# bezirganyan/m2-mixer

Measured on AMD Instinct MI355X. Metric: training samples/sec AV-MNIST M2-Mixer-B bf16, higher is better.
Workload: dtype bf16

## Files before the change

### include/m2mixer.h

```cpp
#ifndef M2MIXER_H
#define M2MIXER_H

#include <stdint.h>

#ifdef __cplusplus
extern "C" {
#endif

#define M2M_ABI_VERSION 18
#define M2M_MAX_BLOCKS 8
#define M2M_ROWS_PER_WG 16

#define M2M_SPLIT_GPART 1472

#define M2M_PREC_BF16 0
#define M2M_PREC_F32 1

typedef struct m2m_block {
    const float* ln1_w;
    const float* ln1_b;
    const float* tok_w1;
    const float* tok_b1;
    const float* tok_w2;
    const float* tok_b2;
// ... 101 lines not shown
int m2m_towers_forward_embeds(const m2m_tower* const* towers, const m2m_tower_io* io, int ntowers,
                              const m2m_embed* const* embeds, const float* const* inputs, const m2m_step_head* head,
                              int B, int training, uint32_t seed, uint32_t step, const uint32_t* step_dev, void* stream);

int m2m_tower_backward(const m2m_tower* t, int B, const float* d_out, int64_t d_out_sample_stride,
                       const float* d_pooled, float* d_x0, int64_t d_x0_sample_stride,
                       uint32_t seed, uint32_t step, const uint32_t* step_dev, void* stream);
typedef struct m2m_tower_gio {
    const float* d_out; int64_t d_out_sample_stride;
    const float* d_pooled;
    float* d_x0; int64_t d_x0_sample_stride;
} m2m_tower_gio;
int m2m_towers_backward(const m2m_tower* const* towers, const m2m_tower_gio* io, int ntowers, int B,
                        uint32_t seed, uint32_t step, const uint32_t* step_dev, void* stream);
int m2m_tower_wgrad(const m2m_tower* t, int B, uint32_t seed, uint32_t step, const uint32_t* step_dev, void* stream);
int m2m_wgrad_form(const m2m_tower* t, int B);
int m2m_split_form(const m2m_tower* a, const m2m_tower* b, int B, int training);
int m2m_towers_wgrad(const m2m_tower* const* towers, const m2m_tower* const* dev_towers, int ntowers,
                     const m2m_embed* const* embeds, const float* const* inputs, const float* const* d_x0s,
                     const m2m_tower* const* embed_towers, int nembeds,
                     int B, uint32_t seed, uint32_t step, const uint32_t* step_dev, void* stream);
int m2m_wgrad_groups(const m2m_tower* t, int B);
int m2m_embeds_wgrad_form(const m2m_embed* const* embeds, const m2m_tower* const* embed_towers, int nembeds, int B);
int m2m_wgrad_slot_groups(const m2m_tower* const* towers, int ntowers, int B);
int m2m_wgrad_fold(const m2m_tower* t, void* stream);
int m2m_embed_wgrad(const m2m_embed* e, const float* input, const float* d_x0, int B, void* stream);
int m2m_embeds_wgrad(const m2m_embed* const* embeds, const float* const* inputs, const float* const* d_x0s, int nembeds, int B,
                     void* stream);

typedef struct m2m_head {
    const float* pooled;
    const float* w;
    const float* b;
    float* g_w;
    float* g_b;
    float* d_pooled;
    float weight;
    float* g_part;
    const float* tokens;
    int64_t tok_sample_stride;
    int32_t ntok;
} m2m_head;
int m2m_heads_part_tiles(int B);
int m2m_heads_ce(const m2m_head* heads, int nheads, const int64_t* labels, int B, int D, int K,
                 float* logits, float* losses, int32_t* preds, int zero_losses, void* stream);

// ... 120 lines not shown
```

### m2_mixer_amd/_lib.py

```python
from __future__ import annotations

import ctypes as C
import os
import subprocess

_HERE = os.path.dirname(os.path.abspath(__file__))
LIB_PATH = os.environ.get("M2M_LIB_PATH", os.path.join(_HERE, "libm2mixer.so"))
CSRC = os.path.join(_HERE, "csrc")

ABI_VERSION = 18
MAX_BLOCKS = 8
ROWS_PER_WG = 16
HCHN_PAD = 4096
SPLIT_ROWS = 128
SPLIT_MAX = 8
SPLIT_GPART = 1472
PREC_BF16, PREC_F32 = 0, 1
PREC_BY_NAME = {"bf16": PREC_BF16, "fp32": PREC_F32, "f32": PREC_F32}

_fp = C.c_void_p


class Block(C.Structure):
    PARAMS = ["ln1_w", "ln1_b", "tok_w1", "tok_b1", "tok_w2", "tok_b2", "ln2_w", "ln2_b",
# ... 89 lines not shown
    "m2m_tower_backward_heads": (C.c_int, [C.POINTER(Tower), C.c_int, C.POINTER(Head), C.c_int, C.c_int, _fp, C.c_int, _fp, _fp, _fp, _fp,
                                           C.c_int64, C.c_uint32, C.c_uint32, _fp, _fp]),
    "m2m_tower_wgrad": (C.c_int, [C.POINTER(Tower), C.c_int, C.c_uint32, C.c_uint32, _fp, _fp]),
    "m2m_towers_can_group": (C.c_int, [C.POINTER(Tower), C.POINTER(Tower), C.c_int]),
    "m2m_towers_forward": (C.c_int, [C.POINTER(C.POINTER(Tower)), C.POINTER(TowerIO), C.c_int, C.c_int, C.c_int, C.c_uint32,
                                     C.c_uint32, _fp, _fp]),
    "m2m_towers_forward_embeds_ok": (C.c_int, [C.POINTER(C.POINTER(Tower)), C.c_int, C.POINTER(C.POINTER(Embed)), C.c_int]),
    "m2m_towers_forward_embeds": (C.c_int, [C.POINTER(C.POINTER(Tower)), C.POINTER(TowerIO), C.c_int, C.POINTER(C.POINTER(Embed)),
                                            C.POINTER(_fp), C.POINTER(StepHead), C.c_int, C.c_int, C.c_uint32, C.c_uint32, _fp, _fp]),
    "m2m_towers_backward": (C.c_int, [C.POINTER(C.POINTER(Tower)), C.POINTER(TowerGIO), C.c_int, C.c_int, C.c_uint32, C.c_uint32,
                                      _fp, _fp]),
    "m2m_towers_wgrad": (C.c_int, [C.POINTER(C.POINTER(Tower)), C.POINTER(_fp), C.c_int, C.POINTER(C.POINTER(Embed)), C.POINTER(_fp),
                                   C.POINTER(_fp), C.POINTER(C.POINTER(Tower)), C.c_int, C.c_int, C.c_uint32, C.c_uint32, _fp, _fp]),
    "m2m_towers_wgrad_heads": (C.c_int, [C.POINTER(C.POINTER(Tower)), C.POINTER(_fp), C.c_int, C.POINTER(C.POINTER(Embed)), C.POINTER(_fp),
                                         C.POINTER(_fp), C.POINTER(C.POINTER(Tower)), C.c_int, C.c_int, C.c_uint32, C.c_uint32, _fp,
                                         C.POINTER(Head), C.c_int, C.c_int, _fp]),
    "m2m_towers_wgrad_tail": (C.c_int, [C.POINTER(C.POINTER(Tower)), C.POINTER(_fp), C.c_int, C.POINTER(C.POINTER(Embed)), C.POINTER(_fp),
                                        C.POINTER(_fp), C.POINTER(C.POINTER(Tower)), C.c_int, C.c_int, C.c_uint32, C.c_uint32, _fp,
                                        C.POINTER(Head), C.c_int, C.c_int, _fp, _fp]),
    "m2m_heads_part_tiles": (C.c_int, [C.c_int]),
    "m2m_wgrad_form": (C.c_int, [C.POINTER(Tower), C.c_int]),
    "m2m_split_form": (C.c_int, [C.POINTER(Tower), C.POINTER(Tower), C.c_int, C.c_int]),
    "m2m_embeds_wgrad_form": (C.c_int, [C.POINTER(C.POINTER(Embed)), C.POINTER(C.POINTER(Tower)), C.c_int, C.c_int]),
    "m2m_wgrad_groups": (C.c_int, [C.POINTER(Tower), C.c_int]),
    "m2m_wgrad_slot_groups": (C.c_int, [C.POINTER(C.POINTER(Tower)), C.c_int, C.c_int]),
    "m2m_wgrad_fold": (C.c_int, [C.POINTER(Tower), _fp]),
    "m2m_adam_step_ranges": (C.c_int, [_fp, _fp, _fp, _fp, _fp, C.c_int64, _fp, C.c_float, C.c_float, C.c_float, C.c_float,
                                       C.c_float, C.c_int, C.POINTER(GradRange), C.c_int, _fp]),
    "m2m_counter_add": (C.c_int, [_fp, C.c_uint32, _fp]),
    "m2m_embed_wgrad": (C.c_int, [C.POINTER(Embed), _fp, _fp, C.c_int, _fp]),
    "m2m_embeds_wgrad": (C.c_int, [C.POINTER(C.POINTER(Embed)), C.POINTER(_fp), C.POINTER(_fp), C.c_int, C.c_int, _fp]),
    "m2m_embeds_forward": (C.c_int, [C.POINTER(C.POINTER(Embed)), C.POINTER(_fp), C.POINTER(_fp), C.POINTER(C.c_int), C.POINTER(C.c_int64),
                                     C.c_int, C.c_int, C.POINTER(StepHead), _fp]),
    "m2m_embed_fwd_splits": (C.c_int, [C.POINTER(Embed)]),
    "m2m_heads_ce": (C.c_int, [C.POINTER(Head), C.c_int, _fp, C.c_int, C.c_int, C.c_int, _fp, _fp, _fp, C.c_int, _fp]),
    "m2m_step_prologue": (C.c_int, [_fp, _fp, _fp, C.c_int, _fp]),
    "m2m_heads_bce": (C.c_int, [C.POINTER(Head), C.c_int, _fp, _fp, C.c_int, C.c_int, C.c_int, _fp, _fp, _fp, C.c_int, _fp]),
    "m2m_heads_ce_w": (C.c_int, [C.POINTER(Head), C.c_int, _fp, C.c_int, C.c_int, C.c_int, _fp, _fp, _fp, C.c_int, _fp, _fp]),
    "m2m_heads_bce_w": (C.c_int, [C.POINTER(Head), C.c_int, _fp, _fp, C.c_int, C.c_int, C.c_int, _fp, _fp, _fp, C.c_int, _fp, _fp]),
    "m2m_fusion_forward": (C.c_int, [C.c_int, _fp, _fp, _fp, C.c_int64, _fp]),
    "m2m_fusion_backward": (C.c_int, [C.c_int, _fp, _fp, _fp, _fp, _fp, C.c_int64, _fp]),
    "m2m_gate_part_floats": (C.c_int64, [C.c_int64, C.c_int]),
    "m2m_gate_forward": (C.c_int, [C.POINTER(Gate), _fp, _fp, _fp, C.c_int64, C.c_int, _fp]),
    "m2m_gate_backward": (C.c_int, [C.POINTER(Gate), _fp, _fp, _fp, C.c_int64, _fp]),
    "m2m_gate_wgrad": (C.c_int, [C.POINTER(Gate), _fp, _fp, C.c_int64, _fp]),
    "m2m_scores_multiclass": (C.c_int, [_fp, _fp, C.c_int, C.c_int, C.c_int, _fp, _fp]),
# ... 91 lines not shown
```

### m2_mixer_amd/csrc/adam.hip

```cpp
#include "dispatch.h"
#include "pack.h"
#include <stdio.h>
#include <string.h>
#include <algorithm>

#define M2M_PACK_TOWERS 3
#define M2M_PACK_EMBEDS 2
struct PackAllArgs {
    m2m_tower4 tw[M2M_PACK_TOWERS];
    m2m_embed em[M2M_PACK_EMBEDS];
    int nt, ne;
    int tile_end[M2M_PACK_TOWERS];
    int embed_wgs0;
    int nt_loads;
    int rowtiles[M2M_PACK_TOWERS];
    int skip_w1tc[M2M_PACK_TOWERS];
};
static_assert(sizeof(PackAllArgs) <= 4096, "kernel arguments are limited to 4 KiB");
static inline int pack_skips_w1tc(const m2m_tower* t) {
    return t->prec == PREC_BF16 && t->D == 128 && !m2m_is_wide(t) && t->slabs == nullptr;
}
extern "C" int m2m_pack_skips_w1tc(const m2m_tower* t) { return t ? pack_skips_w1tc(t) : 0; }

template <int P, bool DO1 = true, bool DO2 = true>
static __device__ __forceinline__ void pack_emit_tile(const m2m_block& k, int D, int q, const float* t1, const float* t2, bool skip_w1tc = false) {
    typedef Prec<P> Pr;
    const int L1 = D + 1, L2 = 33;
    const int tid = threadIdx.x, nthr = blockDim.x;
    const int nKB = D / Pr::KB, nIB = D / 16, CB = 32 / Pr::KB;
    auto emit = [&](char* dst, long blk, int lane, const float (&v)[8]) {
        *reinterpret_cast<u32x4_t*>(dst + (blk * 64 + lane) * 16) = pack_frag<P>(v);
    };
    for (int s = tid; s < 2 * nKB * 64; s += nthr) {
        const int lane = s & 63, bl = s >> 6, h = bl / nKB, kb = bl % nKB, g = lane >> 4, il = lane & 15;
        const int r = 16 * h + il;
        float v1[8], v2[8];
#pragma unroll
        for (int e = 0; e < Pr::EPL; ++e) {
            const int d = kb * Pr::KB + Pr::kmap(PACK_NAT, g, e);
            v1[e] = DO1 ? t1[r * L1 + d] : 0.f;
            v2[e] = DO2 ? t2[d * L2 + r] : 0.f;
        }
        const long blk = (long)(2 * q + h) * nKB + kb;
// ... 746 lines not shown
```

### m2_mixer_amd/csrc/embed_wgrad.h

```cpp
#pragma once
#include "host.h"

#define EBM 32

struct PatchGeom {
    int Cin, H, W, ph, pw, GW, N, K;
};
static __device__ __forceinline__ int patch_koff(const PatchGeom& pg, int k) {
    if (k >= pg.K) return -1;
    const int c = k / (pg.ph * pg.pw), rem = k % (pg.ph * pg.pw);
    const int py = rem / pg.pw, px = rem % pg.pw;
    return (c * pg.H + py) * pg.W + px;
}
static __device__ __forceinline__ long patch_rowbase(const PatchGeom& pg, long m, long M) {
    if (m >= M) return -1;
    const long b = m / pg.N;
    const int n = (int)(m % pg.N);
    const int gy = n / pg.GW, gx = n % pg.GW;
    return (b * pg.Cin * pg.H + gy * pg.ph) * (long)pg.W + gx * pg.pw;
}

template <int P, int D, int NT>
static __device__ __forceinline__ void embed_wgrad_body(const m2m_embed& em, const float* __restrict__ in,
                                                        const float* __restrict__ dx0, long M, int N, int tiles_per_group,
// ... 161 lines not shown
#pragma unroll
            for (int e = 0; e < 8; ++e)
#pragma unroll
                for (int jb = 0; jb < NB; ++jb) t.v[jb][e] = in[rb[e] + (unsigned int)max(ko[jb], 0)];
        }
        t.okbits = 0u;
#pragma unroll
        for (int e = 0; e < 8; ++e) t.okbits |= (okr[e] ? 1u : 0u) << e;
    };
    auto mac = [&](const Tile& t) {
#pragma unroll
        for (int jb = 0; jb < NB; ++jb) {
            Frag b;
            float z[8];
#pragma unroll
            for (int e = 0; e < 8; ++e) z[e] = ((t.okbits >> e) & 1u) && ko[jb] >= 0 ? t.v[jb][e] : 0.f;
#pragma unroll
            for (int e = 0; e < 4; ++e) b.u[e] = pack_bf2(z[2 * e], z[2 * e + 1]);
#pragma unroll
            for (int dt = 0; dt < DT; ++dt) Pr::mma(acc[jb][dt], t.a[dt], b);
        }
    };
    Tile t0, t1;
    const int p0 = wave;
    if (p0 < npairs) load(t0, p0);
    for (int p = p0; p < npairs; p += 2 * NW) {
        if (p + NW < npairs) load(t1, p + NW);
        mac(t0);
        if (p + NW < npairs) {
            if (p + 2 * NW < npairs) load(t0, p + 2 * NW);
            mac(t1);
        }
    }
    f32x4_t* red = reinterpret_cast<f32x4_t*>(smem);
#pragma unroll
    for (int jb = 0; jb < NB; ++jb)
#pragma unroll
        for (int dt = 0; dt < DT; ++dt) red[((wave * NB + jb) * DT + dt) * 64 + lane] = acc[jb][dt];
    __syncthreads();
    for (int q = wave; q < NB * DT; q += NW) {
        const int jb = q / DT, dt = q % DT;
        f32x4_t s = red[q * 64 + lane];
#pragma unroll
        for (int w = 1; w < NW; ++w) s = s + red[(w * NB * DT + q) * 64 + lane];
        const int k = vec2 ? k0 + 2 * il + jb : k0 + 16 * jb + il;
        if (k < em.K) {
            const bool store = (em.wgrad_flags & M2M_WGRAD_OVERWRITE) != 0;
#pragma unroll
            for (int r = 0; r < 4; ++r) {
                float* qd = em.g_w + (long)(16 * dt + 4 * g + r) * em.K + k;
                *qd = store ? s[r] : *qd + s[r];
            }
        }
    }
// ... 121 lines not shown
```

### m2_mixer_amd/csrc/host.h

```cpp
#pragma once
#include "split.h"

void m2m_set_error(const char* msg, const char* file, int line);
int m2m_check_tower(const m2m_tower* t, int B);

static inline int64_t ceil_div(int64_t a, int64_t b) { return (a + b - 1) / b; }



int m2m_check_embed(const m2m_embed* e, int B);

bool m2m_can_group(const m2m_tower* a, const m2m_tower* b);
int m2m_chain_forward_rows(const m2m_tower* t, const float* x0, long x0_ss, int B, float* out, long out_ss, int training,
                           unsigned int seed, unsigned int step, const unsigned int* step_dev, hipStream_t st);
int m2m_chain_forward_rows_group(const m2m_tower* const* v, const float* const* x0, const long* x0_ss, int B, float* const* out,
                                 const long* out_ss, int training, unsigned int seed, unsigned int step, const unsigned int* step_dev,
                                 hipStream_t st);

bool m2m_small_part_deferred(SplitReduceTower& x, const m2m_tower* t, int B);
int m2m_chain_backward_rows(const m2m_tower* t, int B, const float* d_out, long d_out_ss, const float* d_pooled, float* d_x0,
                            long d_x0_ss, unsigned int seed, unsigned int step, const unsigned int* step_dev, hipStream_t st);
int m2m_chain_backward_rows_group(const m2m_tower* const* v, int B, const float* const* d_out, const long* d_out_ss,
                                  const float* const* d_pooled, float* const* d_x0, const long* d_x0_ss, unsigned int seed,
                                  unsigned int step, const unsigned int* step_dev, hipStream_t st);

bool m2m_wgrad_recompute(const m2m_tower* t, int B);

bool m2m_can_group_wide(const m2m_tower* a, const m2m_tower* b, int B);
int m2m_forward_wide(const m2m_tower* t, const float* x0, long x0_ss, int B, float* out, long out_ss, float* pooled,
                     int training, unsigned int seed, unsigned int step, const unsigned int* step_dev, hipStream_t st);
int m2m_backward_wide(const m2m_tower* t, int B, const float* d_out, long d_out_ss, const float* d_pooled, float* d_x0,
                      long d_x0_ss, unsigned int seed, unsigned int step, const unsigned int* step_dev, hipStream_t st);
int m2m_forward_wide_group(const m2m_tower* const* tw, const m2m_tower_io* io, int B, int training, unsigned int seed,
                           unsigned int step, const unsigned int* step_dev, hipStream_t st);
int m2m_backward_wide_group(const m2m_tower* const* tw, const m2m_tower_gio* io, int B, unsigned int seed, unsigned int step,
                            const unsigned int* step_dev, hipStream_t st);

bool m2m_split_eligible(const m2m_tower* t, int B, int training);
bool m2m_split_can_group(const m2m_tower* a, const m2m_tower* b);
int m2m_split_forward(const m2m_tower* const* towers, const m2m_tower_io* io, int ntow, int B, int training, unsigned int seed,
                      unsigned int step, const unsigned int* step_dev, hipStream_t st);
int m2m_split_backward(const m2m_tower* const* towers, const m2m_tower_gio* io, int ntow, int B, unsigned int seed, unsigned int step,
                       const unsigned int* step_dev, hipStream_t st);

int m2m_split_mix_forward(const SplitMixArgs& a, int D, int training, float p_drop, unsigned int seed, unsigned int step,
                          const unsigned int* step_dev, hipStream_t st);
int m2m_split_mix_backward(const SplitMixBwdArgs& a, int D, float p_drop, unsigned int seed, unsigned int step,
                           const unsigned int* step_dev, hipStream_t st);
int m2m_split_small_grads(const SplitReduceArgs& a, hipStream_t st);

int m2m_split_chain_forward(const SplitChainArgs& a, int D, int training, float p_drop, unsigned int seed, unsigned int step,
                            const unsigned int* step_dev, hipStream_t st);
int m2m_split_chain_backward(const SplitChainArgs& a, int D, float p_drop, unsigned int seed, unsigned int step,
                             const unsigned int* step_dev, hipStream_t st);
```

### m2_mixer_amd/csrc/split_api.hip

```cpp
#include "host.h"

static int split_min_rows() { return m2m_env_int("M2M_SPLIT_MIN_ROWS", 1 << 30); }
static int split_mode() { return m2m_env_int("M2M_SPLIT", -1); }

static int split_count(const m2m_tower* t) {
    int s = t->nsplit < SP_MAX_SPLITS ? t->nsplit : SP_MAX_SPLITS;
    const int nunits = t->Cp / 32;
    while (s > 1 && nunits / s < 2) --s;
    return s;
}

bool m2m_split_eligible(const m2m_tower* t, int B, int training) {
    if (split_mode() == 0) return false;
    if (t->prec != PREC_BF16 || m2m_is_wide(t) || t->D != 128 || t->nblocks < 1) return false;
    if (!t->slabs || !t->xres || !t->gpart || split_count(t) < 2) return false;
    for (int b = 0; b < t->nblocks; ++b) {
        if (!t->a_nat[b]) return false;
        if (training && (!t->dy_nat[b] || !t->blk[b].x_in || !t->blk[b].x_mid || !t->blk[b].at_chn)) return false;
    }
    if ((t->Cp / 32 + split_count(t) - 1) / split_count(t) > SP_MAX_UNITS_PER_SPLIT) return false;
    if (split_mode() == 1) return true;
    return (long)B * t->N >= split_min_rows();
}

bool m2m_split_can_group(const m2m_tower* a, const m2m_tower* b) {
    return a->D == b->D && a->p_drop == b->p_drop && (a->N <= 4) == (b->N <= 4) && a->nblocks == b->nblocks &&
           split_count(a) == split_count(b);
}

static void chain_tower(SplitChainTower& c, const m2m_tower* t, int b, int B) {
    const m2m_block& k = t->blk[b];
    c.a_nat = (const char*)t->a_nat[b];
    c.dy_nat = (const char*)t->dy_nat[b];
    c.w1n = (const char*)k.w1n; c.w2c = (const char*)k.w2c; c.w2tn = (const char*)k.w2tn; c.w1tc = (const char*)k.w1tc;
    c.b1p = k.ch_b1p;
    c.slabs = t->slabs;
    c.h_chn = (char*)k.h_chn; c.dh_chn = (char*)k.dh_chn;
    const int SPW = BM / t->N;
    c.M = (B + SPW - 1) / SPW * BM;
    c.rpt = SPW * t->N;
    c.nunits = t->Cp / 32;
    c.Cp = t->Cp;
    c.site = t->site_base + 4u * b + 2u;
    c.p_drop = t->p_drop;
}
// ... 133 lines not shown
```

### m2_mixer_amd/csrc/tower_bwd.hip

```cpp
#include "tile.h"
#include "token_mfma.h"
#include "dispatch.h"
#include <algorithm>

#define BH_MAXH 3
struct BwdHeads {
    m2m_head h[BH_MAXH];
    const int64_t* labels;
    float* logits;
    int32_t* preds;
    int nheads, K, own;
};

template <int P, int D, int NMAX, int TG> struct BwdLds {
    static constexpr bool TOK = NMAX > 0;
    static constexpr int NM = TOK ? NMAX : 1, TW_LD = 2 * NM + 4, XLD = D + 4;
    static constexpr int RED_LD0 = ((32 / TG) * (1 + 2 * NM) + NM) * TG;
    static constexpr int RED_LD = RED_LD0 > TokRed<NM>::LD ? RED_LD0 : TokRed<NM>::LD;
    static constexpr int PB = 4 * D + (TOK ? 32 * TW_LD : 0);
    static constexpr size_t FIXED = (size_t)BM * XLD * sizeof(float) * (1 + RowSlabs<D>::N + 2) + 2 * (size_t)BM * D * Prec<P>::ESZ +
                                    GELU_TAB_N * sizeof(gtabh_t) + (TOK ? (size_t)NWAVES * RED_LD * sizeof(float) : 0);
    static size_t bytes(int nblocks, int N, int Cp) {
        return FIXED + (TOK ? (size_t)(BM / N) * D * sizeof(unsigned int) : 0) + (size_t)nblocks * PB * sizeof(float) +
               (size_t)Cp * sizeof(float) + 16 + 8 * (M2M_MAX_BLOCKS + 1 + BH_MAXH);
// ... 319 lines not shown
#pragma unroll 4
            for (int r = 0; r < BM; ++r) s_ += tdy[r * XLD + d];
            if constexpr (PART) sl_b2[SPP_B2(D) + d] = s_;
            else atomicAdd(reinterpret_cast<float*>((char*)p_gb2) + d, s_);
        }
        pack_tile_chn_t<P, D>(tdy, (char*)p_dyt + pair_off, tile_in_pair, tb1);
        pack_tile_chn_t<P, D>(ta, (char*)p_atc + pair_off, tile_in_pair, tb1);
        if constexpr (HREC) {
            if (tb1 < IMG_B / 16)
                *reinterpret_cast<M2M_AS1 u32x4_t*>(p_h + (long)wg * IMG_B + tb1 * 16) = *reinterpret_cast<const u32x4_t*>(at + tb1 * 16);
        }

        f32x4_t dacc[MT][DT];
#pragma unroll
        for (int mt = 0; mt < MT; ++mt)
#pragma unroll
            for (int dt = 0; dt < DT; ++dt) dacc[mt][dt] = f32x4_t{0.f, 0.f, 0.f, 0.f};
        const int npairs = Cp >> 5;
        asm volatile("" : "+s"(p_w1n), "+s"(p_w2tn), "+s"(p_w1tc), "+s"(p_dh), "+s"(p_h));
        const unsigned int lane16 = (unsigned int)lane * 16u;
        const unsigned int id_sel = (g == (il >> 2)) ? ((il & 1) ? 0x3F800000u : 0x00003F80u) : 0u;
        const unsigned int id_a = (il & 2) ? 0u : id_sel, id_b = (il & 2) ? id_sel : 0u;
        constexpr bool HOLD = D <= 128;
        constexpr bool W1LDS = D == 128 && P == PREC_BF16;
        char* w1slot = reinterpret_cast<char*>(slabs + wave * TILE_F);
        const int swz_w = (il & 7) | ((il & 1) << 3);
        char* w1_wr = w1slot + 256 * il + 16 * (g ^ (swz_w & 3));
        const int rrow = 4 * g + (il >> 2);
        const int swz_r = (rrow & 7) | ((rrow & 1) << 3);
        const char* w1_rd = w1slot + 256 * rrow + 8 * (il & 1) + 16 * (((il >> 1) & 1) ^ (swz_r & 1));
        constexpr bool TICKETS_CT = P == PREC_BF16;
        const bool TICKETS = TICKETS_CT && __builtin_amdgcn_readfirstlane(g_bwd_static_split) == 0;
        TIMER_CRESET();
        constexpr bool STAGED = HOLD && W1LDS && MT == 1 && Act<P>::USES_TABLE && NF == 1;
        f32x4_t bias_n[2] = {f32x4_t{0.f, 0.f, 0.f, 0.f}, f32x4_t{0.f, 0.f, 0.f, 0.f}};
        if constexpr (STAGED) {
            const int q0 = min(TICKETS ? (int)__builtin_amdgcn_readfirstlane(wave) : wave, npairs - 1);
#pragma unroll
            for (int t = 0; t < 2; ++t) bias_n[t] = *reinterpret_cast<const f32x4_t*>(bias_s + 32 * q0 + 16 * t + 4 * g);
        }
        for (int q = __builtin_amdgcn_readfirstlane(wave); q < npairs;) {
            unsigned int ticket = 0u;
            if (TICKETS && lane == 0) ticket = atomicAdd(qctr, 1u);
            if constexpr (STAGED) {
                typedef short s16x4 __attribute__((ext_vector_type(4)));
                typedef unsigned int u32x2 __attribute__((ext_vector_type(2)));
                typedef __attribute__((address_space(3))) s16x4* lds_s16x4_p;
// ... 893 lines not shown
```

### m2_mixer_amd/csrc/tower_wgrad.hip

```cpp
#include "tile.h"
#include "embed_wgrad.h"
#include "dispatch.h"
#include <string.h>

#if defined(__HIP_DEVICE_COMPILE__)
#define M2M_GLOBAL_AS __attribute__((address_space(1)))
#else
#define M2M_GLOBAL_AS
#endif

#define WBM 32
#define WG_RING_MAX 24
#define WG_WAVES 4
#define WG_WAVES_WIDE 5
#define WG_LA 4
#define WG_MINWAVES 2
#define WG_OUT_ATOMIC 0
#define WG_OUT_ADD 1
#define WG_OUT_STORE 2

TIMER_DECL(g_tm_wg);
TIMER_READER(m2m_debug_timers_wgrad, g_tm_wg)

#include "tower_wgrad_rc.h"

template <int P, int D> struct WgradGeom {
// ... 247 lines not shown
    const m2m_block& bk = tw.blk[b];
    WgOut o;
    o.w1 = bk.g_ch_w1; o.w2 = bk.g_ch_w2; o.b1 = bk.g_ch_b1;
    const bool overwrite = (tw.wgrad_flags & M2M_WGRAD_OVERWRITE) != 0;
    if (ngroups == 1) o.mode = overwrite ? WG_OUT_STORE : WG_OUT_ADD;
    else if (slot_mode) {
        if (group == 0) o.mode = overwrite ? WG_OUT_STORE : WG_OUT_ADD;
        else {
            const long cd = (long)tw.C * tw.D;
            float* s = tw.wslot[b];
            o.w1 = s; o.b1 = s + cd; o.w2 = s + cd + tw.C;
            o.mode = WG_OUT_STORE;
        }
    } else o.mode = WG_OUT_ATOMIC;
    return o;
}

template <int P, int D, int RCDM> struct WgradKernelGeom {
    static constexpr bool RC = RCDM >= 0;
    static constexpr int LDS_B = RC ? RcGeom<D>::LDS_B : WgradGeom<P, D>::LDS_B;
    static constexpr int COLS = RC ? RcGeom<D>::COLS : WgradGeom<P, D>::COLS;
    static constexpr int MINWAVES = RC ? 2 : WgradGeom<P, D>::MINWAVES;
    static constexpr int THREADS = RC ? RC_THREADS : WgradGeom<P, D>::THREADS;
};

template <int P, int D, int RCDM, class TW>
static __device__ __forceinline__ void wgrad_dispatch(const TW& tw, int b, int slice, int group, int ngroups, int slot_mode, int ntiles,
                                                      int tpg, int rows_per_t16, unsigned int seed, unsigned int step, char* smem) {
    const WgOut out = wgrad_out(tw, b, group, ngroups, slot_mode);
    if constexpr (RCDM >= 0) {
        const Drop dr = make_drop(true, tw.p_drop, seed, step, tw.site_base + 4u * (unsigned int)b + 2u);
        wgrad_rc_body<D, RCDM>(tw.blk[b], out, tw.Cp, tw.C, slice, group, ntiles, tpg, rows_per_t16, dr.key, dr.scale, smem);
    } else {
        wgrad_body<P, D>(tw.blk[b], out, tw.Cp, tw.C, slice, group, ntiles, tpg, smem);
    }
}

template <int P, int D, int RCDM>
__global__ __launch_bounds__((WgradKernelGeom<P, D, RCDM>::THREADS), (WgradKernelGeom<P, D, RCDM>::MINWAVES)) void tower_wgrad_kernel(
    const m2m_tower tw, int ntiles, int tiles_per_group, int slot_mode, int rows_per_t16, unsigned int seed, unsigned int step_host,
    const unsigned int* __restrict__ step_dev, int dma) {
    extern __shared__ __attribute__((aligned(16))) char smem[];
    const unsigned int step = step_host + (step_dev ? *step_dev : 0u);
    wgrad_dispatch<P, D, RCDM>(tw, (int)blockIdx.y, (int)blockIdx.x, (int)blockIdx.z, (int)gridDim.z, slot_mode, ntiles, tiles_per_group,
                               rows_per_t16, seed, step, smem);
}

#define WG_MAX_TOWERS 4
#define WG_MAX_JOBS 32
struct WgradGroupArgs {
    const m2m_tower* tw[WG_MAX_TOWERS];
    int ntiles[WG_MAX_TOWERS], tpg[WG_MAX_TOWERS], groups[WG_MAX_TOWERS], nsl[WG_MAX_TOWERS], slot[WG_MAX_TOWERS], rpt[WG_MAX_TOWERS];
    unsigned char job_tower[WG_MAX_JOBS], job_block[WG_MAX_JOBS];
    short job_start[WG_MAX_JOBS + 1];
    short xcd_start[8], xcd_len[8];
    int njobs, n_tower_wgs;
    int dma;
    int n_embed_first, n_embed_pad;
    int n_reduce, reduce_sets;
    unsigned int seed, step_host;
    const unsigned int* step_dev;
    unsigned int* bump_counter;
};
template <int P, int D, int RCDM>
__global__ __launch_bounds__((WgradKernelGeom<P, D, RCDM>::THREADS), (WgradKernelGeom<P, D, RCDM>::MINWAVES)) void tower_wgrad_group_kernel(const WgradGroupArgs a,
                                                                                                          const EmbedWgradGroupArgs ea,
                                                                                                          const SplitReduceArgs ra) {
    extern __shared__ __attribute__((aligned(16))) char smem[];
    int id = blockIdx.x;
    if (a.bump_counter && blockIdx.x == 0 && threadIdx.x == 0) *a.bump_counter += 1u;
#ifndef M2M_WG_PROBE_TOWERS_ONLY
    if (a.n_reduce && id >= (int)gridDim.x - a.n_reduce) {
        const int rid = id - ((int)gridDim.x - a.n_reduce);
        const int bx = rid % SPR_NBX, L = (rid / SPR_NBX) % a.reduce_sets, z = rid / (SPR_NBX * a.reduce_sets);
        split_small_grads_body<WgradKernelGeom<P, D, RCDM>::THREADS>(ra.t[z], bx, L, reinterpret_cast<float*>(smem));
        return;
    }
    if (id < a.n_embed_pad) {
        if (id < a.n_embed_first) embed_wgrad_group_body<P, D, WgradKernelGeom<P, D, RCDM>::THREADS>(ea, id, smem);
        return;
    }
    id -= a.n_embed_pad;
    if (id >= a.n_tower_wgs) {
        embed_wgrad_group_body<P, D, WgradKernelGeom<P, D, RCDM>::THREADS>(ea, id - a.n_tower_wgs, smem);
        return;
    }
#endif
    const int xcd = id & 7, idx = id >> 3;
    if (idx >= a.xcd_len[xcd]) return;
    const int lin = a.xcd_start[xcd] + idx;
    int job = 0;
    while (job + 1 < a.njobs && lin >= a.job_start[job + 1]) ++job;
    const int t = a.job_tower[job], rel = lin - a.job_start[job];
    const int slice = rel % a.nsl[t], group = rel / a.nsl[t];
    const m2m_tower& tw = *a.tw[t];
    const unsigned int step = a.step_host + (a.step_dev ? *a.step_dev : 0u);
    wgrad_dispatch<P, D, RCDM>(tw, (int)a.job_block[job], slice, group, a.groups[t], a.slot[t], a.ntiles[t], a.tpg[t], a.rpt[t], a.seed,
                               step, smem);
}

static_assert(sizeof(WgradGroupArgs) + sizeof(EmbedWgradGroupArgs) + sizeof(SplitReduceArgs) <= 3840, "kernel arguments are limited to 4 KiB");

#ifdef M2M_ISA_PROBE
template __global__ void tower_wgrad_group_kernel<PREC_BF16, 128, -1>(const WgradGroupArgs, const EmbedWgradGroupArgs, const SplitReduceArgs);
template __global__ void tower_wgrad_group_kernel<PREC_BF16, 128, DM_HALF>(const WgradGroupArgs, const EmbedWgradGroupArgs, const SplitReduceArgs);
#else
template <int D>
__global__ __launch_bounds__(256, 2) void embed_wgrad_fast_group_kernel(const EmbedWgradGroupArgs ea) {
    extern __shared__ __attribute__((aligned(16))) char smem[];
    embed_wgrad_group_body<PREC_BF16, D, 256>(ea, blockIdx.x, smem);
}

bool m2m_wgrad_recompute(const m2m_tower* t, int B) {
    static const int on = m2m_env_int("M2M_WGRAD_RECOMP", 0);
    if (!on || t->prec != PREC_BF16 || t->D != 128 || t->nblocks < 1 || t->Cp < 64) return false;
    if (m2m_drop_mode(1, t->p_drop) == DM_GEN) return false;
    if (m2m_split_eligible(t, B, 1)) return false;
    return true;
}
extern "C" int m2m_wgrad_form(const m2m_tower* t, int B) { return t && m2m_wgrad_recompute(t, B) ? 1 : 0; }

static bool wgrad_slot_usable(const m2m_tower* t) {
    static const int on = m2m_env_int("M2M_WGRAD_SLOT", 1);
    if (!on || t->nblocks < 1) return false;
    for (int b = 0; b < t->nblocks; ++b) {
        const m2m_block& k = t->blk[b];
        if (!t->wslot[b]) return false;
        if (k.g_ch_b1 != k.g_ch_w1 + (long)t->C * t->D || k.g_ch_w2 != k.g_ch_b1 + t->C) return false;
    }
    return true;
}

struct WgradPlan { int ntiles, nsl, groups, tpg, rpt, slot; };
static WgradPlan wgrad_plan(const m2m_tower* t, int B, int cols, bool honour_overwrite = true) {
    const bool wide = m2m_is_wide(t);
    const int SPW = wide ? 1 : BM / t->N;
    const int nchain = wide ? (int)(((long)B * t->N + BM - 1) / BM) : (B + SPW - 1) / SPW;
    const int ntiles = (nchain * BM + WBM - 1) / WBM;
    const int nsl = (t->Cp + cols - 1) / cols;
    int groups = 1;
    const int wgs = nsl * t->nblocks;
    while (wgs * groups < 128 && (ntiles + groups - 1) / groups > 64) ++groups;
    if (groups < (32 + wgs - 1) / wgs) groups = (32 + wgs - 1) / wgs;
    groups = m2m_env_int("M2M_WGRAD_GROUPS", groups);
    if (ntiles > 64) groups = m2m_env_int("M2M_WGRAD_LONG_GROUPS", groups);
    if (honour_overwrite && (t->wgrad_flags & M2M_WGRAD_OVERWRITE)) groups = 1;
    if (groups < 1) groups = 1;
    int tpg = (ntiles + groups - 1) / groups;
    if (tpg < 4) tpg = 4;
    if (tpg > ntiles) tpg = ntiles;
    groups = (ntiles + tpg - 1) / tpg;
    WgradPlan pl;
    pl.ntiles = ntiles; pl.nsl = nsl; pl.groups = groups; pl.tpg = tpg; pl.slot = 0;
// ... 83 lines not shown
    int n_embed_wgs = 0;
    size_t lds_e = 0;
    bool embeds_separately = false;
    if (nembeds) {
        n_embed_wgs = (P == PREC_BF16 && nembeds == EMB_GROUP) ? embed_wgrad_group_args_fast(ea, embeds, inputs, embed_towers, B) : 0;
        if (n_embed_wgs) lds_e = embed_wgrad_fast_lds<D, KG::THREADS>();
        else if (KG::THREADS == 256) { static const int ewgs = m2m_env_int("M2M_EMBED_WGS", D >= 256 ? 128 : 512);    n_embed_wgs = embed_wgrad_group_args(ea, embeds, inputs, d_x0s, B, ewgs, nembeds); lds_e = embed_wgrad_lds<D, P>(); }
        else embeds_separately = true;
    }
    if (embeds_separately) {
        if (nembeds == 1) { if (int rc = m2m_embed_wgrad(embeds[0], inputs[0], d_x0s[0], B, (void*)st)) return rc; }
        else if (int rc = m2m_embeds_wgrad(embeds, inputs, d_x0s, nembeds, B, (void*)st)) return rc;
    }
    if constexpr (P == PREC_BF16) {
        static const int merged = m2m_env_int("M2M_EMBED_MERGED", 1);
        if (n_embed_wgs && ea.fast && !merged && KG::THREADS != 256) {
            const size_t le = embed_wgrad_fast_lds<D, 256>();
            if (int rc = m2m_launch<embed_wgrad_fast_group_kernel<D>>(dim3((unsigned)n_embed_wgs), dim3(256), le, le, st, ea)) return rc;
            n_embed_wgs = 0; lds_e = 0;
        }
    }
    const size_t lds_t = (size_t)KG::LDS_B;
    const size_t lds = lds_t > lds_e ? lds_t : lds_e;
    static const int embed_first = m2m_env_int("M2M_EMBED_FIRST", 1);
    if (ea.fast && n_embed_wgs && embed_first) { a.n_embed_first = n_embed_wgs; a.n_embed_pad = (n_embed_wgs + 7) & ~7; n_embed_wgs = 0; }
    SplitReduceArgs ra;
    memset(&ra, 0, sizeof(ra));
    for (int i = 0; i < n; ++i) {
        if (!(host[i]->wgrad_flags & M2M_WGRAD_REDUCES_SMALL)) continue;
        SplitReduceTower x;
        if (!m2m_small_part_deferred(x, host[i], B)) continue;
        if (ra.ntow < SPR_MAX_TOWERS && KG::THREADS % SPR_COLS == 0) { ra.t[ra.ntow++] = x; continue; }
        SplitReduceArgs one;
        memset(&one, 0, sizeof(one));
        one.t[0] = x; one.ntow = 1;
        if (int rc = m2m_split_small_grads(one, st)) return rc;
    }
    if (heads_reduce) {
        if (ra.ntow < SPR_MAX_TOWERS && KG::THREADS % SPR_COLS == 0) ra.t[ra.ntow++] = *heads_reduce;
        else {
            SplitReduceArgs one;
            memset(&one, 0, sizeof(one));
            one.t[0] = *heads_reduce; one.ntow = 1;
            if (int rc = m2m_split_small_grads(one, st)) return rc;
        }
    }
    for (int i = 0; i < ra.ntow; ++i) a.reduce_sets = ra.t[i].nlaunch > a.reduce_sets ? ra.t[i].nlaunch : a.reduce_sets;
    a.n_reduce = SPR_NBX * a.reduce_sets * ra.ntow;
    return m2m_launch<tower_wgrad_group_kernel<P, D, RCDM>>(dim3((unsigned)(a.n_embed_pad + a.n_tower_wgs + n_embed_wgs + a.n_reduce)), dim3(KG::THREADS),
                                                            lds, lds, st, a, ea, ra);
}

extern "C" int m2m_wgrad_slot_groups(const m2m_tower* const* towers, int ntowers, int B) {
    if (!towers || ntowers < 1 || ntowers > WG_MAX_TOWERS) return 0;
    WgradPlan pl[WG_MAX_TOWERS];
    wgrad_group_plans(towers, ntowers, B, wgrad_cols(towers[0], B), pl);
    int bits = 0;
    for (int i = 0; i < ntowers; ++i) bits |= pl[i].slot << i;
    return bits;
}

extern "C" int m2m_tower_wgrad(const m2m_tower* t, int B, uint32_t seed, uint32_t step, const uint32_t* step_dev, void* stream) {
    if (int rc = m2m_check_tower(t, B)) return rc;
    if (t->nblocks == 0) return 0;
    hipStream_t st = reinterpret_cast<hipStream_t>(stream);
    if (t->wgrad_flags & M2M_WGRAD_REDUCES_SMALL) {
        SplitReduceArgs one;
        memset(&one, 0, sizeof(one));
        if (m2m_small_part_deferred(one.t[0], t, B)) {
            one.ntow = 1;
            if (int rc = m2m_split_small_grads(one, st)) return rc;
// ... 83 lines not shown
extern "C" int m2m_towers_wgrad_heads(const m2m_tower* const* towers, const m2m_tower* const* dev_towers, int ntowers,
                                      const m2m_embed* const* embeds, const float* const* inputs, const float* const* d_x0s,
                                      const m2m_tower* const* embed_towers, int nembeds,
                                      int B, uint32_t seed, uint32_t step, const uint32_t* step_dev,
                                      const m2m_head* heads, int nheads, int K, void* stream) {
    return towers_wgrad_impl(towers, dev_towers, ntowers, embeds, inputs, d_x0s, embed_towers, nembeds, B, seed, step, step_dev, heads, nheads, K, stream);
}

extern "C" int m2m_towers_wgrad_tail(const m2m_tower* const* towers, const m2m_tower* const* dev_towers, int ntowers,
                                     const m2m_embed* const* embeds, const float* const* inputs, const float* const* d_x0s,
                                     const m2m_tower* const* embed_towers, int nembeds,
                                     int B, uint32_t seed, uint32_t step, const uint32_t* step_dev,
                                     const m2m_head* heads, int nheads, int K, uint32_t* bump_counter, void* stream) {
    return towers_wgrad_impl(towers, dev_towers, ntowers, embeds, inputs, d_x0s, embed_towers, nembeds, B, seed, step, step_dev, heads, nheads, K, stream, bump_counter);
}

extern "C" int m2m_embeds_wgrad_form(const m2m_embed* const* embeds, const m2m_tower* const* embed_towers, int nembeds, int B) {
    if (!embeds || !embed_towers || nembeds != EMB_GROUP) return 0;
    EmbedWgradGroupArgs ea;
    const float* ins[EMB_GROUP] = {nullptr, nullptr};
    return embed_wgrad_group_args_fast(ea, embeds, ins, embed_towers, B) > 0 ? 1 : 0;
}

__global__ void wgrad_fold_kernel(float* __restrict__ g, const float* __restrict__ s, long n) {
    const long stride = (long)gridDim.x * blockDim.x;
    for (long i = (long)blockIdx.x * blockDim.x + threadIdx.x; i < n; i += stride) g[i] += s[i];
}
extern "C" int m2m_wgrad_fold(const m2m_tower* t, void* stream) {
    if (!t) { m2m_set_error("wgrad_fold: null tower", __FILE__, __LINE__); return -1; }
    if (!wgrad_slot_usable(t)) { m2m_set_error("wgrad_fold: channel gradients are not contiguous", __FILE__, __LINE__); return -1; }
    hipStream_t st = reinterpret_cast<hipStream_t>(stream);
    const long n = 2L * t->C * t->D + t->C;
    for (int b = 0; b < t->nblocks; ++b) {
        if (int rc = m2m_launch<wgrad_fold_kernel>(dim3(512), dim3(256), 0, 0, st, t->blk[b].g_ch_w1, t->wslot[b], n)) return rc;
    }
    return 0;
}
#endif
```

Baseline: 1.044 million.

## Schedule embed and reduce wgrad units via atomic ticket queue

Replaces the static assignment of embed-wgrad and small-grad reduce workgroups with a dynamic ticket queue. Spare workgroups sized to idle CUs, plus tower-wgrad workgroups once their main job ends, pull units from a per-stream global atomic counter. The aim is to fill idle CUs and absorb load imbalance at the tail of the fused wgrad kernel. It also software-pipelines the embed-wgrad load/mac loop by clamping indices rather than branching, and tightens the W1^T skip predicate. The cost is extra atomics, global counter state that must reset correctly, and per-stream slot bookkeeping on the host.

Result: no change. 1.037 million (-0.7%).

```diff
diff --git a/include/m2mixer.h b/include/m2mixer.h
--- a/include/m2mixer.h
+++ b/include/m2mixer.h
@@ -147,6 +147,8 @@
                      int B, uint32_t seed, uint32_t step, const uint32_t* step_dev, void* stream);
 int m2m_wgrad_groups(const m2m_tower* t, int B);
 int m2m_embeds_wgrad_form(const m2m_embed* const* embeds, const m2m_tower* const* embed_towers, int nembeds, int B);
+int m2m_wgrad_ticket_form(const m2m_tower* const* towers, int ntowers, const m2m_embed* const* embeds,
+                          const m2m_tower* const* embed_towers, int nembeds, int B);
 int m2m_wgrad_slot_groups(const m2m_tower* const* towers, int ntowers, int B);
 int m2m_wgrad_fold(const m2m_tower* t, void* stream);
 int m2m_embed_wgrad(const m2m_embed* e, const float* input, const float* d_x0, int B, void* stream);
diff --git a/m2_mixer_amd/_lib.py b/m2_mixer_amd/_lib.py
--- a/m2_mixer_amd/_lib.py
+++ b/m2_mixer_amd/_lib.py
@@ -135,6 +135,7 @@
     "m2m_wgrad_form": (C.c_int, [C.POINTER(Tower), C.c_int]),
     "m2m_split_form": (C.c_int, [C.POINTER(Tower), C.POINTER(Tower), C.c_int, C.c_int]),
     "m2m_embeds_wgrad_form": (C.c_int, [C.POINTER(C.POINTER(Embed)), C.POINTER(C.POINTER(Tower)), C.c_int, C.c_int]),
+    "m2m_wgrad_ticket_form": (C.c_int, [C.POINTER(C.POINTER(Tower)), C.c_int, C.POINTER(C.POINTER(Embed)), C.POINTER(C.POINTER(Tower)), C.c_int, C.c_int]),
     "m2m_wgrad_groups": (C.c_int, [C.POINTER(Tower), C.c_int]),
     "m2m_wgrad_slot_groups": (C.c_int, [C.POINTER(C.POINTER(Tower)), C.c_int, C.c_int]),
     "m2m_wgrad_fold": (C.c_int, [C.POINTER(Tower), _fp]),
diff --git a/m2_mixer_amd/csrc/adam.hip b/m2_mixer_amd/csrc/adam.hip
--- a/m2_mixer_amd/csrc/adam.hip
+++ b/m2_mixer_amd/csrc/adam.hip
@@ -17,8 +17,10 @@
     int skip_w1tc[M2M_PACK_TOWERS];
 };
 static_assert(sizeof(PackAllArgs) <= 4096, "kernel arguments are limited to 4 KiB");
+static_assert(m2m_bwd_parks_w1(PREC_BF16, 128) && !m2m_bwd_parks_w1(PREC_F32, 128) && !m2m_bwd_parks_w1(PREC_BF16, 64) && !m2m_bwd_parks_w1(PREC_BF16, 256),
+              "pack_skips_w1tc: exactly the bf16 / hidden_dim 128 backward does without the W1^T copy");
 static inline int pack_skips_w1tc(const m2m_tower* t) {
-    return t->prec == PREC_BF16 && t->D == 128 && !m2m_is_wide(t) && t->slabs == nullptr;
+    return m2m_bwd_parks_w1(t->prec, t->D) && !m2m_is_wide(t) && !m2m_split_possible(t);
 }
 extern "C" int m2m_pack_skips_w1tc(const m2m_tower* t) { return t ? pack_skips_w1tc(t) : 0; }
 
diff --git a/m2_mixer_amd/csrc/embed_wgrad.h b/m2_mixer_amd/csrc/embed_wgrad.h
--- a/m2_mixer_amd/csrc/embed_wgrad.h
+++ b/m2_mixer_amd/csrc/embed_wgrad.h
@@ -207,14 +207,14 @@
         }
     };
     Tile t0, t1;
-    const int p0 = wave;
-    if (p0 < npairs) load(t0, p0);
-    for (int p = p0; p < npairs; p += 2 * NW) {
-        if (p + NW < npairs) load(t1, p + NW);
-        mac(t0);
-        if (p + NW < npairs) {
-            if (p + 2 * NW < npairs) load(t0, p + 2 * NW);
-            mac(t1);
+    const int p0 = wave, plast = npairs - 1;
+    if (p0 < npairs) {
+        load(t0, p0);
+        for (int p = p0; p < npairs; p += 2 * NW) {
+            load(t1, min(p + NW, plast));
+            mac(t0);
+            load(t0, min(p + 2 * NW, plast));
+            if (p + NW < npairs) mac(t1);
         }
     }
     f32x4_t* red = reinterpret_cast<f32x4_t*>(smem);
diff --git a/m2_mixer_amd/csrc/host.h b/m2_mixer_amd/csrc/host.h
--- a/m2_mixer_amd/csrc/host.h
+++ b/m2_mixer_amd/csrc/host.h
@@ -17,6 +17,7 @@
                                  const long* out_ss, int training, unsigned int seed, unsigned int step, const unsigned int* step_dev,
                                  hipStream_t st);
 
+constexpr bool m2m_bwd_parks_w1(int prec, int D) { return D == 128 && prec == PREC_BF16; }
 bool m2m_small_part_deferred(SplitReduceTower& x, const m2m_tower* t, int B);
 int m2m_chain_backward_rows(const m2m_tower* t, int B, const float* d_out, long d_out_ss, const float* d_pooled, float* d_x0,
                             long d_x0_ss, unsigned int seed, unsigned int step, const unsigned int* step_dev, hipStream_t st);
@@ -37,6 +38,7 @@
                             const unsigned int* step_dev, hipStream_t st);
 
 bool m2m_split_eligible(const m2m_tower* t, int B, int training);
+bool m2m_split_possible(const m2m_tower* t);
 bool m2m_split_can_group(const m2m_tower* a, const m2m_tower* b);
 int m2m_split_forward(const m2m_tower* const* towers, const m2m_tower_io* io, int ntow, int B, int training, unsigned int seed,
                       unsigned int step, const unsigned int* step_dev, hipStream_t st);
diff --git a/m2_mixer_amd/csrc/split_api.hip b/m2_mixer_amd/csrc/split_api.hip
--- a/m2_mixer_amd/csrc/split_api.hip
+++ b/m2_mixer_amd/csrc/split_api.hip
@@ -10,7 +10,7 @@
     return s;
 }
 
-bool m2m_split_eligible(const m2m_tower* t, int B, int training) {
+static bool split_tower_ok(const m2m_tower* t, int training) {
     if (split_mode() == 0) return false;
     if (t->prec != PREC_BF16 || m2m_is_wide(t) || t->D != 128 || t->nblocks < 1) return false;
     if (!t->slabs || !t->xres || !t->gpart || split_count(t) < 2) return false;
@@ -19,8 +19,18 @@
         if (training && (!t->dy_nat[b] || !t->blk[b].x_in || !t->blk[b].x_mid || !t->blk[b].at_chn)) return false;
     }
     if ((t->Cp / 32 + split_count(t) - 1) / split_count(t) > SP_MAX_UNITS_PER_SPLIT) return false;
+    return true;
+}
+
+bool m2m_split_eligible(const m2m_tower* t, int B, int training) {
+    if (!split_tower_ok(t, training)) return false;
     if (split_mode() == 1) return true;
     return (long)B * t->N >= split_min_rows();
+}
+
+bool m2m_split_possible(const m2m_tower* t) {
+    if (!split_tower_ok(t, 0)) return false;
+    return split_mode() == 1 || split_min_rows() < (1 << 30);
 }
 
 bool m2m_split_can_group(const m2m_tower* a, const m2m_tower* b) {
diff --git a/m2_mixer_amd/csrc/tower_bwd.hip b/m2_mixer_amd/csrc/tower_bwd.hip
--- a/m2_mixer_amd/csrc/tower_bwd.hip
+++ b/m2_mixer_amd/csrc/tower_bwd.hip
@@ -365,7 +365,8 @@
         const unsigned int id_sel = (g == (il >> 2)) ? ((il & 1) ? 0x3F800000u : 0x00003F80u) : 0u;
         const unsigned int id_a = (il & 2) ? 0u : id_sel, id_b = (il & 2) ? id_sel : 0u;
         constexpr bool HOLD = D <= 128;
-        constexpr bool W1LDS = D == 128 && P == PREC_BF16;
+        constexpr bool W1LDS = m2m_bwd_parks_w1(P, D);
+        static_assert(W1LDS == (D == 128 && P == PREC_BF16), "the W1 slot holds 256-byte rows of bf16; the re-pack skips W1^T by the same predicate");
         char* w1slot = reinterpret_cast<char*>(slabs + wave * TILE_F);
         const int swz_w = (il & 7) | ((il & 1) << 3);
         char* w1_wr = w1slot + 256 * il + 16 * (g ^ (swz_w & 3));
diff --git a/m2_mixer_amd/csrc/tower_wgrad.hip b/m2_mixer_amd/csrc/tower_wgrad.hip
--- a/m2_mixer_amd/csrc/tower_wgrad.hip
+++ b/m2_mixer_amd/csrc/tower_wgrad.hip
@@ -2,6 +2,8 @@
 #include "embed_wgrad.h"
 #include "dispatch.h"
 #include <string.h>
+#include <mutex>
+#include <vector>
 
 #if defined(__HIP_DEVICE_COMPILE__)
 #define M2M_GLOBAL_AS __attribute__((address_space(1)))
@@ -295,6 +297,7 @@
     static constexpr int COLS = RC ? RcGeom<D>::COLS : WgradGeom<P, D>::COLS;
     static constexpr int MINWAVES = RC ? 2 : WgradGeom<P, D>::MINWAVES;
     static constexpr int THREADS = RC ? RC_THREADS : WgradGeom<P, D>::THREADS;
+    static constexpr bool TICKETS = !RC && P == PREC_BF16 && WgradGeom<P, D>::WAVES == WG_WAVES_WIDE;
 };
 
 template <int P, int D, int RCDM, class TW>
@@ -317,6 +320,33 @@
     const unsigned int step = step_host + (step_dev ? *step_dev : 0u);
     wgrad_dispatch<P, D, RCDM>(tw, (int)blockIdx.y, (int)blockIdx.x, (int)blockIdx.z, (int)gridDim.z, slot_mode, ntiles, tiles_per_group,
                                rows_per_t16, seed, step, smem);
+}
+
+#define WG_TICKET_SLOTS 64
+static __device__ unsigned int g_wg_ticket[WG_TICKET_SLOTS][2];
+
+template <int P, int D, int NT, class A>
+static __device__ __forceinline__ void wgrad_tickets(const A& a, const EmbedWgradGroupArgs& ea, const SplitReduceArgs& ra, char* smem) {
+    __shared__ unsigned int s_unit;
+    unsigned int* ctr = g_wg_ticket[a.ticket_slot];
+    const unsigned int n_embed = (unsigned int)a.n_embed_units, n_units = n_embed + (unsigned int)a.n_reduce_units;
+    for (;;) {
+        __syncthreads();
+        if (threadIdx.x == 0) s_unit = atomicAdd(ctr, 1u);
+        __syncthreads();
+        const unsigned int u = (unsigned int)__builtin_amdgcn_readfirstlane((int)s_unit);
+        if (u >= n_units) break;
+        if (u < n_embed) embed_wgrad_group_body<P, D, NT>(ea, (int)u, smem);
+        else {
+            const int rid = (int)(u - n_embed);
+            const int bx = rid % SPR_NBX, L = (rid / SPR_NBX) % a.reduce_sets, z = rid / (SPR_NBX * a.reduce_sets);
+            split_small_grads_body<NT>(ra.t[z], bx, L, reinterpret_cast<float*>(smem));
+        }
+    }
+    if (threadIdx.x == 0) {
+        __threadfence();
+        if (atomicAdd(ctr + 1, 1u) == (unsigned int)a.n_ticket_wgs - 1u) { atomicExch(ctr, 0u); atomicExch(ctr + 1, 0u); }
+    }
 }
 
 #define WG_MAX_TOWERS 4
@@ -334,6 +364,7 @@
     unsigned int seed, step_host;
     const unsigned int* step_dev;
     unsigned int* bump_counter;
+    int ticket_slot, n_embed_units, n_reduce_units, n_ticket_wgs;
 };
 template <int P, int D, int RCDM>
 __global__ __launch_bounds__((WgradKernelGeom<P, D, RCDM>::THREADS), (WgradKernelGeom<P, D, RCDM>::MINWAVES)) void tower_wgrad_group_kernel(const WgradGroupArgs a,
@@ -349,8 +380,15 @@
         split_small_grads_body<WgradKernelGeom<P, D, RCDM>::THREADS>(ra.t[z], bx, L, reinterpret_cast<float*>(smem));
         return;
     }
+    constexpr bool TK = WgradKernelGeom<P, D, RCDM>::TICKETS;
     if (id < a.n_embed_pad) {
-        if (id < a.n_embed_first) embed_wgrad_group_body<P, D, WgradKernelGeom<P, D, RCDM>::THREADS>(ea, id, smem);
+        if (id < a.n_embed_first) {
+            bool spare = false;
+            if constexpr (TK) {
+                if (a.ticket_slot >= 0) { spare = true; wgrad_tickets<P, D, WgradKernelGeom<P, D, RCDM>::THREADS>(a, ea, ra, smem); }
+            }
+            if (!spare) embed_wgrad_group_body<P, D, WgradKernelGeom<P, D, RCDM>::THREADS>(ea, id, smem);
+        }
         return;
     }
     id -= a.n_embed_pad;
@@ -370,6 +408,11 @@
     const unsigned int step = a.step_host + (a.step_dev ? *a.step_dev : 0u);
     wgrad_dispatch<P, D, RCDM>(tw, (int)a.job_block[job], slice, group, a.groups[t], a.slot[t], a.ntiles[t], a.tpg[t], a.rpt[t], a.seed,
                                step, smem);
+#ifndef M2M_WG_PROBE_TOWERS_ONLY
+    if constexpr (WgradKernelGeom<P, D, RCDM>::TICKETS) {
+        if (a.ticket_slot >= 0) wgrad_tickets<P, D, WgradKernelGeom<P, D, RCDM>::THREADS>(a, ea, ra, smem);
+    }
+#endif
 }
 
 static_assert(sizeof(WgradGroupArgs) + sizeof(EmbedWgradGroupArgs) + sizeof(SplitReduceArgs) <= 3840, "kernel arguments are limited to 4 KiB");
@@ -402,6 +445,28 @@
         if (k.g_ch_b1 != k.g_ch_w1 + (long)t->C * t->D || k.g_ch_w2 != k.g_ch_b1 + t->C) return false;
     }
     return true;
+}
+
+static int wgrad_ticket_slot(hipStream_t st) {
+    static std::mutex mu;
+    static std::vector<hipStream_t> seen;
+    std::lock_guard<std::mutex> lock(mu);
+    for (size_t i = 0; i < seen.size(); ++i)
+        if (seen[i] == st) return (int)i;
+    if (seen.size() >= WG_TICKET_SLOTS) return -1;
+    seen.push_back(st);
+    return (int)seen.size() - 1;
+}
+static int wgrad_embed_first() { static const int on = m2m_env_int("M2M_EMBED_FIRST", 1); return on; }
+static int wgrad_tickets_on() { static const int on = m2m_env_int("M2M_EMBED_TICKETS", 1); return on; }
+static int wgrad_cu_count() {
+    static std::mutex mu;
+    static int cus[64];
+    int dev = 0;
+    if (hipGetDevice(&dev) != hipSuccess || dev < 0 || dev >= 64) return 256;
+    std::lock_guard<std::mutex> lock(mu);
+    if (!cus[dev] && hipDeviceGetAttribute(&cus[dev], hipDeviceAttributeMultiprocessorCount, dev) != hipSuccess) cus[dev] = 256;
+    return cus[dev] > 0 ? cus[dev] : 256;
 }
 
 struct WgradPlan { int ntiles, nsl, groups, tpg, rpt, slot; };
@@ -531,8 +596,17 @@
     }
     const size_t lds_t = (size_t)KG::LDS_B;
     const size_t lds = lds_t > lds_e ? lds_t : lds_e;
-    static const int embed_first = m2m_env_int("M2M_EMBED_FIRST", 1);
-    if (ea.fast && n_embed_wgs && embed_first) { a.n_embed_first = n_embed_wgs; a.n_embed_pad = (n_embed_wgs + 7) & ~7; n_embed_wgs = 0; }
+    const int embed_first = wgrad_embed_first();
+    a.ticket_slot = -1;
+    bool tickets = false;
+    if constexpr (KG::TICKETS) {
+        if (ea.fast && n_embed_wgs && embed_first && wgrad_tickets_on()) {
+            a.ticket_slot = wgrad_ticket_slot(st);
+            tickets = a.ticket_slot >= 0;
+        }
+    }
+    if (tickets) { a.n_embed_units = n_embed_wgs; n_embed_wgs = 0; }
+    else if (ea.fast && n_embed_wgs && embed_first) { a.n_embed_first = n_embed_wgs; a.n_embed_pad = (n_embed_wgs + 7) & ~7; n_embed_wgs = 0; }
     SplitReduceArgs ra;
     memset(&ra, 0, sizeof(ra));
     for (int i = 0; i < n; ++i) {
@@ -556,6 +630,15 @@
     }
     for (int i = 0; i < ra.ntow; ++i) a.reduce_sets = ra.t[i].nlaunch > a.reduce_sets ? ra.t[i].nlaunch : a.reduce_sets;
     a.n_reduce = SPR_NBX * a.reduce_sets * ra.ntow;
+    if (tickets) {
+        a.n_reduce_units = a.n_reduce;
+        a.n_reduce = 0;
+        const int cus = wgrad_cu_count(), units = a.n_embed_units + a.n_reduce_units;
+        int spare = total < cus ? cus - total : 8;
+        if (spare > units) spare = units;
+        a.n_embed_first = spare; a.n_embed_pad = (spare + 7) & ~7;
+        a.n_ticket_wgs = spare + total;
+    }
     return m2m_launch<tower_wgrad_group_kernel<P, D, RCDM>>(dim3((unsigned)(a.n_embed_pad + a.n_tower_wgs + n_embed_wgs + a.n_reduce)), dim3(KG::THREADS),
                                                             lds, lds, st, a, ea, ra);
 }
@@ -685,6 +768,17 @@
     return embed_wgrad_group_args_fast(ea, embeds, ins, embed_towers, B) > 0 ? 1 : 0;
 }
 
+static_assert(WgradKernelGeom<PREC_BF16, 128, -1>::TICKETS && !WgradKernelGeom<PREC_BF16, 64, -1>::TICKETS && !WgradKernelGeom<PREC_F32, 128, -1>::TICKETS &&
+              !WgradKernelGeom<PREC_BF16, 128, DM_NONE>::TICKETS, "m2m_wgrad_ticket_form restates WgradKernelGeom::TICKETS");
+extern "C" int m2m_wgrad_ticket_form(const m2m_tower* const* towers, int ntowers, const m2m_embed* const* embeds,
+                                     const m2m_tower* const* embed_towers, int nembeds, int B) {
+    if (!towers || ntowers < 1 || !towers[0]) return 0;
+    const m2m_tower* t = towers[0];
+    if (t->prec != PREC_BF16 || t->D != 128 || m2m_wgrad_recompute(t, B)) return 0;
+    if (!m2m_embeds_wgrad_form(embeds, embed_towers, nembeds, B)) return 0;
+    return wgrad_embed_first() && wgrad_tickets_on() ? 1 : 0;
+}
+
 __global__ void wgrad_fold_kernel(float* __restrict__ g, const float* __restrict__ s, long n) {
     const long stride = (long)gridDim.x * blockDim.x;
     for (long i = (long)blockIdx.x * blockDim.x + threadIdx.x; i < n; i += stride) g[i] += s[i];
```
